# magic-research/vector_quantization

Measured on AMD Instinct MI355X. Metric: quantized tokens/sec, VQGAN quantizer forward K=16384 D=256, higher is better.
Workload: dtype f16+f32; 1 GPU; VQGAN K=16384 D=256, 256x256 images -> 16x16 tokens, bf16 latents, VQGANQuantizer.forward of the drop-in nn.Module, eval mode (prepare+argmin+gather+STE+loss); images_per_gpu=2048, parallelism=dp1 (independent shards, no data-path collective)

## Files before the change

vector_quantization_amd/csrc/vqhip.hip:

```cpp
#include "vqhip.h"

#include <hip/hip_runtime.h>
#include <stdio.h>
#include <string.h>

#include "vqhip_host.h"
#include "vqhip_kernels.h"
#include "vqhip_prepare_kernels.h"
#include "vqhip_proposal_kernels.h"
#include "vqhip_refine_kernels.h"
#include "vqhip_proposal32_kernels.h"
#include "vqhip_exact_kernels.h"
#include "vqhip_stream_kernels.h"
#include "vqhip_update_kernels.h"
#include "vqhip_sort_kernels.h"
#include "vqhip_aux_kernels.h"
#include "vqhip_exchange_kernels.h"
#include "vqhip_step_kernels.h"
#include "vqhip_pool_kernels.h"
#include "vqhip_fsq_kernels.h"

#include <atomic>
#include <mutex>
#include <type_traits>
#include <vector>
static std::atomic<bool> g_prof_on{false};
static std::mutex g_prof_mu;
static std::vector<std::pair<hipEvent_t, hipEvent_t>> g_prof_events;
static size_t g_prof_used = 0;

static long prof_begin(hipStream_t s) {
    if (!g_prof_on.load(std::memory_order_relaxed)) return -1;
    std::lock_guard<std::mutex> lock(g_prof_mu);
    if (g_prof_used == g_prof_events.size()) {
        hipEvent_t a, b;
        if (hipEventCreate(&a) != hipSuccess || hipEventCreate(&b) != hipSuccess) { g_prof_on = false; return -1; }
        g_prof_events.emplace_back(a, b);
    }
    const long slot = (long)g_prof_used++;
    (void)hipEventRecord(g_prof_events[slot].first, s);
    return slot;
}
static void prof_end(long slot, hipStream_t s) {
    if (slot < 0) return;
    std::lock_guard<std::mutex> lock(g_prof_mu);
    if ((size_t)slot < g_prof_events.size()) (void)hipEventRecord(g_prof_events[slot].second, s);
}

static std::atomic<int> g_tune_slices{0};
static std::atomic<int> g_tune_force_exact{0};
static std::atomic<int> g_tune_stream{1};
#define VQ_FUSED_DECIDE_MAX_N 16384

template <int NSTEP, int TT, int WAVES, int TPS, int NBUF = 2, bool FILTER = false, bool NOAUX = false, bool GROUPS = false, int XD = 0>
static int launch_coarse_cfg(const char *ximg, int64_t N, const char *frag, int64_t nstages, int nslices, float *rec,
                             int64_t Np, const VqCbStats *cbst, const float *xh2, const float *rho2, int Dp, int metric,
                             const VqDecideOut &dec, int pad_stage, int tpb, hipStream_t s) {
    constexpr int LDS = NBUF * (TPS * NSTEP + VQ_AUX_CHUNKS(TPS)) * VQ_CHUNK_BYTES;
    auto kern = coarse_kernel<NSTEP, TT, WAVES, TPS, NBUF, FILTER, NOAUX, GROUPS, XD>;
    static LdsCache lds_set;
    if (int rc = ensure_dyn_lds((const void *)kern, LDS, lds_set)) return rc;
    const int64_t ntiles = (N + 15) / 16;
    const int64_t ntb = (ntiles + tpb - 1) / tpb;
    const int grid = (int)(ntb * nslices);
    const long slot = prof_begin(s);
    kern<<<grid, WAVES * 64, LDS, s>>>(ximg, N, frag, nstages, nslices, rec, Np, cbst, xh2, rho2, Dp, metric, dec, pad_stage, tpb);
    prof_end(slot, s);
    VQ_CHECK_LAUNCH("coarse_kernel");
    return VQHIP_OK;
}

template <int TT, int WAVES, int TPS, int NBUF, bool NOAUX, int KS>
static int launch_coarse32_cfg(const char *ximg, int64_t N, const char *frag, int64_t nstages, int nslices, float *rec,
                               int64_t Np, const VqCbStats *cbst, const float *xh2, const float *rho2, int Dp, int metric,
                               const int *n_dev, const VqGroupLists &grp, int pad_stage, int tpb, hipStream_t s) {
    constexpr int LDS = NBUF * (TPS * 2 + VQ_AUX_CHUNKS(TPS)) * VQ_CHUNK_BYTES;
    auto kern = coarse32_kernel<TT, WAVES, TPS, NBUF, NOAUX, KS, VQ_GROUP_TILES>;
    static LdsCache lds_set;
    if (int rc = ensure_dyn_lds((const void *)kern, LDS, lds_set)) return rc;
    const int64_t ntiles = (N + 15) / 16;
    const int64_t ntb = (ntiles + tpb - 1) / tpb;
    const long slot = prof_begin(s);
    kern<<<(int)(ntb * nslices), WAVES * 64, LDS, s>>>(ximg, N, frag, nstages, nslices, rec, Np, cbst, xh2, rho2, Dp, metric, n_dev, grp, pad_stage, tpb);
    prof_end(slot, s);
    VQ_CHECK_LAUNCH("coarse32_kernel");
    return VQHIP_OK;
}

template <int NSTEP, int TT, int WAVES, int TPS, int NBUF = 2, int XD = 0>
static int launch_rescan_cfg(const char *ximg, const char *frag, int64_t nstages, const int *rescan_list, const int *counters,
                             const float *thr, int *rescan_cnt, int *cand_list, hipStream_t s, const void *xrows = nullptr) {
    constexpr int LDS = NBUF * (TPS * NSTEP + VQ_AUX_CHUNKS(TPS)) * VQ_CHUNK_BYTES + WAVES * TT * 16 * 4 * (1 + VQ_RESCAN_LOCAL);
    auto kern = rescan_kernel<NSTEP, TT, WAVES, TPS, NBUF, XD>;
    static LdsCache lds_set;
    if (int rc = ensure_dyn_lds((const void *)kern, LDS, lds_set)) return rc;
    kern<<<256, WAVES * 64, LDS, s>>>(ximg, frag, nstages, rescan_list, counters, thr, rescan_cnt, cand_list, xrows);
    VQ_CHECK_LAUNCH("rescan_kernel");
    return VQHIP_OK;
}

#ifndef VQ_W32_MAX_D
#define VQ_W32_MAX_D 32
#endif
#ifndef VQ_NBUF_D32
#define VQ_NBUF_D32 4
#endif
#ifndef VQ_D32_SMALL_TT
#define VQ_D32_SMALL_TT 2
#define VQ_D32_SMALL_W 8
#endif
#ifndef VQ_MIN_SLICES_FILTER
#define VQ_MIN_SLICES_FILTER 1
#endif
static int balanced_tiles_per_block(int64_t N, int full) {
    if (full < 16) return full;
    const int64_t ntiles = (N + 15) / 16;
    int best = full;
    int64_t best_cost = ((ntiles + full - 1) / full + 255) / 256 * full;
    for (int tpb = full - 1; tpb >= full / 2 && tpb >= 8; --tpb) {
        const int64_t cost = ((ntiles + tpb - 1) / tpb + 255) / 256 * tpb;
        if (cost < best_cost) { best_cost = cost; best = tpb; }
    }
    return best;
}

static bool vq_xdirect(int64_t N, int64_t K, int D, int x_dtype, int metric, const int *n_dev) {
    if (D != 256 || n_dev != nullptr || vq_cb_layout(K, D).nstages < 2 || g_tune_slices.load() == 1) return false;
    if (x_dtype != VQHIP_DTYPE_BF16) return false;
    if (!vq_public_metric(metric)) return false;
    if (N <= VQ_FUSED_DECIDE_MAX_N) return false;
    return !(N <= 4096 || (N <= 256 * 64 && K <= 4096));
}
enum VqTokenSide { VQ_TOKENS_UNPREPARED, VQ_TOKENS_IMAGE, VQ_TOKENS_ROWS };

static int pick_slices(int64_t ntb, int64_t nstages, int min_slices = 2) {
    if (const int forced = g_tune_slices.load(); forced > 0) { int ns = forced; while (ns > 1 && ns > nstages) ns >>= 1; return ns; }
    int64_t want = (256 + ntb - 1) / ntb;
    want = want < min_slices ? min_slices : want;
    int ns = 1;
    while (ns < want && ns < VQ_MAX_SLICES) ns <<= 1;
    while (ns > 1 && ns > nstages) ns >>= 1;
    return ns;
}

struct VqGroupRun { int used, ks, noaux, pad_stage; };
static int launch_coarse(const char *ximg, int64_t N, const VqCbLayout &L, const char *frag, float *rec, int64_t Np,
                         const VqCbStats *cbst, const float *xh2, const float *rho2, int metric, const VqDecideOut &dec,
                         int *nslices_out, int *fused_decide_out, hipStream_t s, VqGroupLists grp = VqGroupLists{nullptr, nullptr, nullptr, nullptr, 0, 1, 0},
                         VqGroupRun *grun = nullptr, bool xd = false) {
    const int nstep = L.nstep;
    const bool small = N <= 256 * 64;
    const bool small16 = N <= 4096 || (N <= 256 * 64 && L.K <= 4096);
    const bool small32 = N < 512 * 512;
    const bool noaux = !VQ_IS_L2(metric);
    const int pad_stage = (L.K % ((int64_t)L.tps * VQ_TILE_CODES)) ? (int)(L.nstages - 1) : -1;
#define VQ_CFG(NS, TT, W, ...)                                                                      \
    {                                                                                               \
        int64_t ntb = (N + (W) * (TT) * 16 - 1) / ((W) * (TT) * 16);                                \
        int ns = pick_slices(ntb, L.nstages, (NS) <= 8 ? VQ_MIN_SLICES_FILTER : 2);                 \
        *nslices_out = ns;                                                                          \
        const int tpb = (ns == 1) ? balanced_tiles_per_block(N, (W) * (TT)) : (W) * (TT);           \
        VqDecideOut dsel = dec;                                                                     \
        if (!(ns == 1 || N <= VQ_FUSED_DECIDE_MAX_N)) dsel.idx = nullptr;                           \
        *fused_decide_out = dsel.idx != nullptr ? 1 : 0;                                            \
        return launch_coarse_cfg<NS, TT, W, __VA_ARGS__>(ximg, N, frag, L.nstages, ns, rec, Np, cbst, xh2, rho2, L.Dp, metric, dsel, pad_stage, tpb, s); \
    }
    switch (nstep) {
        case 2: if ((L.D <= 16 || (L.D <= VQ_W32_MAX_D && noaux)) && N >= VQ_W32_MIN_N && grp.bcnt != nullptr && grun != nullptr) {
                    const int tt = small32 ? 1 : 2;
                    const int full = 8 * tt * 2;
                    const int64_t ntb0 = (N + full * 16 - 1) / (full * 16);
                    int ns = pick_slices(ntb0, L.nstages, VQ_MIN_SLICES_FILTER);
                    ns = ns > VQ_GROUP_MAX_SLICES ? VQ_GROUP_MAX_SLICES : ns;
                    *nslices_out = ns;
                    int tpb = (ns == 1) ? balanced_tiles_per_block(N, full) : full;
                    tpb = (tpb + 1) & ~1;
                    *fused_decide_out = 0;
                    grun->used = 1; grun->ks = L.D <= 16 ? 1 : 2; grun->noaux = noaux ? 1 : 0; grun->pad_stage = pad_stage;
#define VQ_CFG32(TTW, NOAUXV, KSV) return launch_coarse32_cfg<TTW, 8, VQ_TPS_D32, VQ_NBUF_D32, NOAUXV, KSV>(ximg, N, frag, L.nstages, ns, rec, Np, cbst, xh2, rho2, L.Dp, metric, dec.n_dev, grp, pad_stage, tpb, s)
                    if (L.D <= 16) {
                        if (tt == 1) { if (noaux) VQ_CFG32(1, true, 1); else VQ_CFG32(1, false, 1); }
                        else { if (noaux) VQ_CFG32(2, true, 1); else VQ_CFG32(2, false, 1); }
                    } else {
                        if (tt == 1) { if (noaux) VQ_CFG32(1, true, 2); else VQ_CFG32(1, false, 2); }
                        else { if (noaux) VQ_CFG32(2, true, 2); else VQ_CFG32(2, false, 2); }
                    }
#undef VQ_CFG32
                }
                if (N >= VQ_GROUPS_MIN_N) {
                    if (noaux) { if (small32) VQ_CFG(2, VQ_D32_SMALL_TT, VQ_D32_SMALL_W, VQ_TPS_D32, VQ_NBUF_D32, true, true, true) else VQ_CFG(2, 4, 8, VQ_TPS_D32, VQ_NBUF_D32, true, true, true) }
                    if (small32) VQ_CFG(2, VQ_D32_SMALL_TT, VQ_D32_SMALL_W, VQ_TPS_D32, VQ_NBUF_D32, true, false, true) else VQ_CFG(2, 4, 8, VQ_TPS_D32, VQ_NBUF_D32, true, false, true)
                }
                if (noaux) { if (small32) VQ_CFG(2, VQ_D32_SMALL_TT, VQ_D32_SMALL_W, VQ_TPS_D32, VQ_NBUF_D32, true, true) else VQ_CFG(2, 4, 8, VQ_TPS_D32, VQ_NBUF_D32, true, true) }
                if (small32) VQ_CFG(2, VQ_D32_SMALL_TT, VQ_D32_SMALL_W, VQ_TPS_D32, VQ_NBUF_D32, true) else VQ_CFG(2, 4, 8, VQ_TPS_D32, VQ_NBUF_D32, true)
        case 4: if (small) VQ_CFG(4, 2, 8, 4, 4, true) else VQ_CFG(4, 4, 8, 4, 4, true)
        case 8: if (small) VQ_CFG(8, 2, 8, 4, 4, true) else VQ_CFG(8, 4, 8, 4, 4, true)
        case 16: if (xd && !small16) VQ_CFG(16, 4, 8, VQ_TPS16, 4, false, false, false, 1)
                 if (small16) VQ_CFG(16, 2, 8, VQ_TPS16, 4) else VQ_CFG(16, 4, 8, VQ_TPS16, 4)
        case 32: VQ_CFG(32, 2, 8, 2)
        case 48: VQ_CFG(48, 2, 8, 1)
        case 64: {
            auto cost = [&](int tokens, double eff) {
                const int64_t ntb = (N + tokens - 1) / tokens;
                const int ns = pick_slices(ntb, L.nstages, 2);
                return (double)((ntb * ns + 255) / 256) * tokens * ((double)L.nstages / ns) / eff;
            };
            if (cost(192, 1.18) < cost(128, 1.0)) VQ_CFG(64, 3, 4, 1) else VQ_CFG(64, 1, 8, 1)
        }
        default: break;
    }
#undef VQ_CFG
    return fail(VQHIP_EINVAL, "vqhip_argmin: unsupported padded D");
}

static int resident_grid(int per_cu) {
    static std::atomic<int> cus[VQ_MAX_DEVICES];
    int dev = 0, n = 0;
    if (hipGetDevice(&dev) != hipSuccess) return 256 * per_cu;
    if (dev >= 0 && dev < VQ_MAX_DEVICES && (n = cus[dev].load(std::memory_order_relaxed)) > 0) return n * per_cu;
    if (hipDeviceGetAttribute(&n, hipDeviceAttributeMultiprocessorCount, dev) != hipSuccess || n <= 0) n = 256;
    if (dev >= 0 && dev < VQ_MAX_DEVICES) cus[dev].store(n, std::memory_order_relaxed);
    return n * per_cu;
}

template <int MODE>
static int run_exact_tiled(const void *x, int x_dtype, const float *e, const float *en, const float *xn, int64_t N, int64_t K,
                           int D, int metric, u64 *keys, float *dout, hipStream_t s) {
    const int bf = x_dtype == VQHIP_DTYPE_F32 ? 0 : 1;
    const int64_t items = ((N + 127) / 128) * ((K + 255) / 256);
    if (g_tune_stream.load() && D % (bf ? 8 : 4) == 0 && items < (int64_t)1 << 31) {
        static LdsCache ssets[2];
        const int lds = vq_xs_lds_bytes(bf);
        const void *kern = bf ? (const void *)exact_stream_kernel<1, MODE> : (const void *)exact_stream_kernel<0, MODE>;
        if (int rc = ensure_dyn_lds(kern, lds, ssets[bf])) return rc;
        const int cap = resident_grid(2);
        const int grid = (int)(items < cap ? items : cap);
        if (bf) exact_stream_kernel<1, MODE><<<grid, 256, lds, s>>>(x, e, en, xn, N, K, D, metric, keys, dout);
        else exact_stream_kernel<0, MODE><<<grid, 256, lds, s>>>(x, e, en, xn, N, K, D, metric, keys, dout);
        VQ_CHECK_LAUNCH("exact_stream_kernel");
        return VQHIP_OK;
    }
    constexpr int LDS = 2 * 32 * 128 * 4 + 8 * 32 * 4;
    static LdsCache sets[4];
    const void *kerns[4] = {(const void *)exact_tiled_kernel<0, MODE, false>, (const void *)exact_tiled_kernel<1, MODE, false>,
                            (const void *)exact_tiled_kernel<0, MODE, true>, (const void *)exact_tiled_kernel<1, MODE, true>};
    const int v4 = (D % 4 == 0) ? 2 : 0;
    if (int rc = ensure_dyn_lds(kerns[v4 + bf], LDS, sets[v4 + bf])) return rc;
    int grid = (int)(items < 1024 ? items : 1024);
#define VQ_TILED(DT, V4) exact_tiled_kernel<DT, MODE, V4><<<grid, 256, LDS, s>>>(x, e, en, xn, N, K, D, metric, keys, dout)
    if (v4) { if (bf) VQ_TILED(1, true); else VQ_TILED(0, true); }
    else { if (bf) VQ_TILED(1, false); else VQ_TILED(0, false); }
#undef VQ_TILED
    VQ_CHECK_LAUNCH("exact_tiled_kernel");
    return VQHIP_OK;
}

template <int MODE>
static int exact_whole(const void *x, int x_dtype, const float *e, int64_t N, int64_t K, int D, int metric, const VqWsView &V,
                       int64_t *idx, float *dmin, int32_t *hist, float *dout, hipStream_t s) {
    constexpr bool keyed = MODE != 2;
    const bool l2 = metric == VQHIP_METRIC_L2;
    if (l2) if (int rc = vqhip_row_sqnorm(e, VQHIP_DTYPE_F32, K, D, V.en, s)) return rc;
    if constexpr (keyed) { fill_u64_kernel<<<256, 256, 0, s>>>(V.keys, N, ~0ull); VQ_CHECK_LAUNCH("fill_u64_kernel"); }
    if (l2) if (int rc = vqhip_row_sqnorm(x, x_dtype, N, D, V.xn_whole, s)) return rc;
    if (int rc = run_exact_tiled<MODE>(x, x_dtype, e, V.en, V.xn_whole, N, K, D, metric, keyed ? V.keys : nullptr, dout, s)) return rc;
    if constexpr (keyed) { finalize_kernel<<<256, 256, 0, s>>>(V.keys, nullptr, nullptr, N, idx, dmin, hist); VQ_CHECK_LAUNCH("finalize_kernel"); }
    return VQHIP_OK;
}

static int exact_few_max(int D) {
    if (D > 512 || D > VQ_FEW_MAX_D) return 0;
    static std::atomic<int> lds_limit{-1};
    int lim = lds_limit.load(std::memory_order_relaxed);
    if (lim < 0) {
        int dev = 0, v = 0;
        if (hipGetDevice(&dev) != hipSuccess || hipDeviceGetAttribute(&v, hipDeviceAttributeMaxSharedMemoryPerBlock, dev) != hipSuccess) v = 65536;
        lim = v;
        lds_limit.store(lim);
    }
    return vq_few_lds_bytes(D) <= lim ? VQ_EXACT_FEW_MAX : 0;
}

static int run_exact_rows(const void *x, int x_dtype, const float *e, const float *en, const float *xn, int64_t N, int64_t K, int D,
                          int metric, const int *row_list, const int *nrows_dev, u64 *keys, int *ticket, int64_t *idx,
                          int32_t *hist, hipStream_t s) {
    const int64_t ncb = (K + 63) / 64;
    const int grid = (int)(ncb < 256 ? 256 : (ncb > 1024 ? 1024 : ncb));
    if (D % 4) return fail(VQHIP_EINVAL, "exact_kernel: D % 4 != 0 (the proposal route has D % 8 == 0)");
    const int few_max = exact_few_max(D);
    const int lds = few_max ? vq_few_lds_bytes(D) : 0;
    static LdsCache sets[2];
    const int bf = x_dtype == VQHIP_DTYPE_F32 ? 0 : 1;
    if (int rc = ensure_dyn_lds(bf ? (const void *)exact_kernel<1> : (const void *)exact_kernel<0>, lds, sets[bf])) return rc;
    if (!bf)
        exact_kernel<0><<<grid, 256, lds, s>>>(x, e, en, xn, N, K, D, metric, row_list, nrows_dev, keys, ticket, idx, hist, few_max);
    else
        exact_kernel<1><<<grid, 256, lds, s>>>(x, e, en, xn, N, K, D, metric, row_list, nrows_dev, keys, ticket, idx, hist, few_max);
    VQ_CHECK_LAUNCH("exact_kernel");
    return VQHIP_OK;
}

template <int MODE>
static int run_segsum(const void *src, int x_dtype, const float *e, const int64_t *idx, const int32_t *order,
                      const int32_t *offsets, int64_t N, int64_t K, int D, const float *g_cb, float *dst, void *ws,
                      hipStream_t s) {
    float *partial = (float *)ws;
    const int64_t nranges = (N + VQ_SEG_RANGE - 1) / VQ_SEG_RANGE;
    int grid = (int)((nranges + 3) / 4); grid = grid < 1 ? 1 : (grid > 4096 ? 4096 : grid);
    if (x_dtype == VQHIP_DTYPE_F32) segsum_rows_kernel<MODE, 0><<<grid, 256, 0, s>>>(src, e, idx, order, offsets, N, (int)K, D, g_cb, dst, partial);
    else segsum_rows_kernel<MODE, 1><<<grid, 256, 0, s>>>(src, e, idx, order, offsets, N, (int)K, D, g_cb, dst, partial);
    VQ_CHECK_LAUNCH("segsum_rows_kernel");
    int fgrid = (int)((K + 3) / 4); fgrid = fgrid > 2048 ? 2048 : fgrid;
    segsum_fixup_kernel<<<fgrid, 256, 0, s>>>(offsets, (int)K, D, partial, dst);
    VQ_CHECK_LAUNCH("segsum_fixup_kernel");
    return VQHIP_OK;
}

static inline int vq_small_lanes(int D) { return D <= 8 ? 8 : (D <= 16 ? 16 : 32); }

template <bool NORMALIZE>
static int launch_row_small(const void *v, int dtype, int64_t R, int D, float eps, float *out, hipStream_t s) {
    const int L = vq_small_lanes(D);
    const int grid = waves_grid((R + 64 / L - 1) / (64 / L), 4);
#define VQ_ROW_SMALL(DT, LL) row_small_kernel<DT, LL, NORMALIZE><<<grid, 256, 0, s>>>(v, R, D, eps, out)
    if (dtype == VQHIP_DTYPE_F32) { if (L == 8) VQ_ROW_SMALL(0, 8); else if (L == 16) VQ_ROW_SMALL(0, 16); else VQ_ROW_SMALL(0, 32); }
    else { if (L == 8) VQ_ROW_SMALL(1, 8); else if (L == 16) VQ_ROW_SMALL(1, 16); else VQ_ROW_SMALL(1, 32); }
#undef VQ_ROW_SMALL
    VQ_CHECK_LAUNCH("row_small_kernel");
    return VQHIP_OK;
}

template <typename IdxT>
static int launch_hist(const IdxT *idx, int64_t N, int64_t K, int32_t *hist, void *stream) {
    constexpr bool i64 = sizeof(IdxT) == 8;
    VQ_REQUIRE(idx && hist && N >= 0 && K > 0, i64 ? "vqhip_hist: bad argument" : "vqhip_hist_i32: bad argument");
    if (N == 0) return VQHIP_OK;
    hipStream_t s = (hipStream_t)stream;
    if (K <= 32768 && N >= 16384) {
        static LdsCache lds_set;
        if (int rc = ensure_dyn_lds(i64 ? (const void *)hist_lds_kernel : (const void *)hist_i32_lds_kernel, (size_t)K * 4, lds_set)) return rc;
        int grid = (int)((N + 2047) / 2048); grid = grid > 256 ? 256 : grid;
        if constexpr (i64) hist_lds_kernel<<<grid, 1024, (size_t)K * 4, s>>>(idx, N, (int)K, hist);
        else hist_i32_lds_kernel<<<grid, 1024, (size_t)K * 4, s>>>(idx, N, (int)K, hist);
    } else {
        int grid = (int)((N + 255) / 256); grid = grid > 2048 ? 2048 : grid;
        if constexpr (i64) hist_kernel<<<grid, 256, 0, s>>>(idx, N, K, hist);
        else hist_i32_kernel<<<grid, 256, 0, s>>>(idx, N, K, hist);
    }
    VQ_CHECK_LAUNCH(i64 ? "hist_kernel" : "hist_i32_kernel");
    return VQHIP_OK;
// ... 1285 lines not shown
```

vector_quantization_amd/csrc/vqhip_proposal_kernels.h:

```cpp
#pragma once
#include "vqhip_kernels.h"
struct Top2 { float v1, v2, v3; uint32_t c1, c2; };
__device__ __forceinline__ float row_margin(const VqCbStats *st, int Dp, int metric, float X2, float R2, float *bf16_part = nullptr);

struct VqDecideOut {
    int64_t *idx; int32_t *hist;
    int *rescan_list, *multi_list, *exact_list, *counters;
    u64 *keys; float *thr_out; int *rescan_cnt;
    int *arrive;
    const int *n_dev;
    const void *xrows; float *xh2_w, *rho2_w, *xn_w;
};
template <bool AGENT>
__device__ __forceinline__ void decide_rows(int64_t n, bool oob, const VqCbStats *st, int Dp, int metric, int nslices,
                                            const float *rec, const float *xh2, const float *rho2, int64_t Np,
                                            const VqDecideOut &o, int *wcount, int *wbase, const float *rece2 = nullptr);

__device__ __forceinline__ void top_insert(Top2 &t, float v, uint32_t c) {
    if (v > t.v1) { t.v3 = fmaxf(t.v3, t.v2); t.v2 = t.v1; t.c2 = t.c1; t.v1 = v; t.c1 = c; }
    else if (v > t.v2) { t.v3 = fmaxf(t.v3, t.v2); t.v2 = v; t.c2 = c; }
    else t.v3 = fmaxf(t.v3, v);
}

__device__ __forceinline__ void top_merge_lane(Top2 &t, int xor_mask) {
    Top2 o;
    o.v1 = __shfl_xor(t.v1, xor_mask, 64); o.v2 = __shfl_xor(t.v2, xor_mask, 64); o.v3 = __shfl_xor(t.v3, xor_mask, 64);
    o.c1 = __shfl_xor(t.c1, xor_mask, 64); o.c2 = __shfl_xor(t.c2, xor_mask, 64);
    if (o.c1 != 0xFFFFFFFFu) top_insert(t, o.v1, o.c1);
    if (o.c2 != 0xFFFFFFFFu) top_insert(t, o.v2, o.c2);
    t.v3 = fmaxf(t.v3, o.v3);
}

__device__ __forceinline__ int tile_row16(int e, int lane) { return 16 * (e >> 2) + 4 * (lane >> 4) + (e & 3); }

#ifndef VQ_D32_PLAIN_OCC
#define VQ_D32_PLAIN_OCC 2
#endif
template <int NSTEP, int TT, int WAVES, int TPS, int NBUF = 2, bool FILTER = false, bool NOAUX = false,
          bool GROUPS = false, int XD = 0>
__global__ __launch_bounds__(WAVES * 64, (FILTER && NSTEP <= 2) ? (GROUPS ? 4 : VQ_D32_PLAIN_OCC) : WAVES / 4) void coarse_kernel(
    const char *__restrict__ ximg, int64_t N, const char *__restrict__ frag, int64_t nstages, int nslices,
    float *__restrict__ rec, int64_t Np, const VqCbStats *__restrict__ cbst, const float *__restrict__ xh2,
    const float *__restrict__ rho2, int Dp, int metric, VqDecideOut dec, int pad_stage, int tpb) {
    extern __shared__ __attribute__((aligned(16))) char lds[];
    static_assert(NSTEP % 2 == 0, "16x16x32 layout: 32-dim k-steps");
    static_assert(!GROUPS || FILTER, "group records are a form of the filtered epilogue");
    constexpr bool GBRANCH = TT >= VQ_GROUP_BRANCH_MIN_TT;
    constexpr bool PIPE = (TPS % 2) == 0;
    constexpr bool PIPE_H = (TPS == 1) && (WAVES <= 4);
    static_assert(!(PIPE_H && (NOAUX || FILTER)), "half-tile ping-pong: plain large-D form only");
    constexpr int NS32 = NSTEP / 2;
    constexpr int NCH = TPS * NSTEP + VQ_AUX_CHUNKS(TPS);
    constexpr int STAGE_BYTES = NCH * VQ_CHUNK_BYTES;
    constexpr int NE = 8;
#ifndef VQ_SCALAR_WAVE
#define VQ_SCALAR_WAVE 1
#endif
    const int lane = threadIdx.x & 63;
    const int wave = (VQ_SCALAR_WAVE && NSTEP > 2) ? __builtin_amdgcn_readfirstlane((int)(threadIdx.x >> 6)) : (int)(threadIdx.x >> 6);
    const int64_t ntt = (N + 31) / 32 * 2;
    if (dec.n_dev != nullptr) {
        const int64_t nd = *dec.n_dev;
        N = nd < N ? nd : N;
        if ((int64_t)(blockIdx.x / nslices) * tpb * 16 >= N) return;
    }
    const bool wave_active = wave * TT < tpb;
    cb_stats_publish(cbst);
    const int sl = blockIdx.x % nslices;
    const int64_t tb = blockIdx.x / nslices;
    const int64_t st0 = (nstages * sl) / nslices, st1 = (nstages * (sl + 1)) / nslices;
  for (bool once = true; once; once = false) {

    half8 xf[TT][NS32];
    if constexpr (XD == 0) {
#pragma unroll
        for (int t = 0; t < TT; ++t) {
            int64_t tt = tb * tpb + wave * TT + t;
            tt = tt < ntt ? tt : ntt - 1;
            const char *src = ximg + tt * (int64_t)(NS32 * VQ_CHUNK_BYTES) + lane * 16;
#pragma unroll
            for (int s = 0; s < NS32; ++s) xf[t][s] = *(const half8 *)(src + s * VQ_CHUNK_BYTES);
        }
    } else {
        static_assert(XD == 1 && !FILTER && !GROUPS && !NOAUX && (NSTEP % 4) == 0, "token side in the prologue: bf16 rows, plain D % 64 == 0 forms");
        const int q4 = lane >> 4, r16 = lane & 15;
        constexpr int Dr = NS32 * 32;
        static_assert(NS32 == 8 && NBUF >= 4 && 2 * STAGE_BYTES >= WAVES * 16 * 528, "row tile: D = 256, staged behind stage 1");
        char *stg = lds + 2 * STAGE_BYTES + wave * (16 * 528);
        const int hr = lane >> 5, c32 = lane & 31;
#pragma unroll
        for (int t = 0; t < TT; ++t) {
            const int64_t tok0 = (tb * tpb + wave * TT + t) * 16;
#pragma unroll
            for (int i = 0; i < 8; ++i) {
                const int64_t tok = tok0 + 2 * i + hr;
                const int64_t trow = tok < N ? tok : N - 1;
                xf[t][i] = *(const half8 *)((const uint16_t *)dec.xrows + trow * Dr + 8 * c32);
            }
        }
        __builtin_amdgcn_sched_barrier(0);
#pragma unroll
        for (int t = 0; t < TT; ++t) {
#pragma unroll
            for (int i = 0; i < 8; ++i) *(half8 *)(stg + (2 * i + hr) * 528 + 16 * c32) = xf[t][i];
#pragma unroll
            for (int s = 0; s < NS32; ++s) xf[t][s] = *(const half8 *)(stg + r16 * 528 + 64 * s + 16 * q4);
        }
#pragma unroll
        for (int t = 0; t < TT; ++t) {
            const int64_t tok = (tb * tpb + wave * TT + t) * 16 + r16;
            [[maybe_unused]] const int64_t trow = tok < N ? tok : N - 1;
            const bool stats = sl == 0;
            float sh[2] = {0.0f, 0.0f}, sr[2] = {0.0f, 0.0f}, pn[2][8];
#pragma unroll
            for (int j = 0; j < 8; ++j) { pn[0][j] = 0.0f; pn[1][j] = 0.0f; }
#pragma unroll
            for (int s = 0; s < NS32; ++s) {
                float v[8];
                half8 f;
                typedef uint32_t u32x4 __attribute__((ext_vector_type(4)));
                typedef _Float16 half2v __attribute__((ext_vector_type(2)));
                typedef float float2v __attribute__((ext_vector_type(2)));
                const u32x4 bits = __builtin_bit_cast(u32x4, xf[t][s]);
#pragma unroll
                for (int j = 0; j < 4; ++j) {
                    const uint32_t lo = bits[j] << 16, hi = bits[j] & 0xFFFF0000u;
                    v[2 * j] = __uint_as_float(lo); v[2 * j + 1] = __uint_as_float(hi);
                    float2v c;
                    c[0] = (lo & 0x7FFFFFFFu) < 0x38800000u ? 0.0f : v[2 * j];
                    c[1] = (hi & 0x7FFFFFFFu) < 0x38800000u ? 0.0f : v[2 * j + 1];
                    const half2v h = __builtin_convertvector(c, half2v);
                    f[2 * j] = h[0]; f[2 * j + 1] = h[1];
                }
                if (stats) {
#pragma unroll
                    for (int j = 0; j < 8; ++j) {
                        const float b = (float)f[j], res = v[j] - b;
                        sh[s & 1] = fmaf(b, b, sh[s & 1]); sr[s & 1] = fmaf(res, res, sr[s & 1]);
                        pn[s & 1][j] = fmaf(v[j], v[j], pn[s & 1][j]);
                    }
                }
                xf[t][s] = f;
            }
            if (!stats) continue;
            float a = 0.0f, b = 0.0f;
#pragma unroll
            for (int g = 0; g < 8; ++g) {
                a += __shfl(sh[g >> 2], (g & 3) * 16 + r16, 64);
                b += __shfl(sr[g >> 2], (g & 3) * 16 + r16, 64);
            }
            float q[8];
#pragma unroll
            for (int j = 0; j < 8; ++j) q[j] = pn[0][j] + pn[1][j];
#pragma unroll
            for (int j = 0; j < 8; ++j) q[j] = q[j] + __shfl_xor(q[j], 32, 64);
#pragma unroll
            for (int j = 0; j < 8; ++j) q[j] = q[j] + __shfl_xor(q[j], 16, 64);
            float a0 = q[0] + q[4], a1 = q[1] + q[5], a2 = q[2] + q[6], a3 = q[3] + q[7];
            a0 = a0 + a2; a1 = a1 + a3;
            a0 = a0 + a1;
            if (sl == 0 && q4 == 0 && tok < N && wave * TT + t < tpb) { dec.xh2_w[tok] = a; dec.rho2_w[tok] = b; dec.xn_w[tok] = a0; }
        }
    }
    if constexpr (PIPE_H) {
#pragma unroll
        for (int t = 0; t < TT; ++t)
#pragma unroll
            for (int s = 0; s < NS32; ++s) {
                if (t >= TT / 2) asm volatile("" : "+a"(xf[t][s]));
                else asm volatile("" : "+v"(xf[t][s]));
            }
    }

    float b1[TT], b2[TT], th[TT], mg[TT];
    uint32_t t1[TT];
#pragma unroll
    for (int t = 0; t < TT; ++t) { b1[t] = -INFINITY; b2[t] = -INFINITY; th[t] = -INFINITY; mg[t] = INFINITY; t1[t] = 0; }
    static_assert(!FILTER || PIPE, "the filtered epilogue is written for the ping-pong form");
    float sc0 = 0.0f, sc1 = 0.0f, sc2 = 0.0f;
    if constexpr (FILTER) {
        const VqCbStats stv = cb_stats_view(cbst);
#pragma unroll
        for (int t = 0; t < TT; ++t) {
            int64_t tokn = (tb * tpb + wave * TT + t) * 16 + (lane & 15);
            tokn = tokn < N ? tokn : N - 1;
            const float m = row_margin(&stv, Dp, metric, xh2[tokn], rho2[tokn]);
            mg[t] = (m > 0.0f) ? m : INFINITY;
        }
    }

    auto issue_stage = [&](int64_t st, int buf) {
        const char *src = frag + st * (int64_t)STAGE_BYTES;
        char *dstb = lds + buf * STAGE_BYTES;
        for (int c = wave; c < NCH; c += WAVES)
            __builtin_amdgcn_global_load_lds(
                (const __attribute__((address_space(1))) void *)(src + c * VQ_CHUNK_BYTES + lane * 16),
                (__attribute__((address_space(3))) void *)(dstb + c * VQ_CHUNK_BYTES), 16, 0, 0);
    };

    constexpr int AHEAD = NBUF >= 3 ? 2 : 1;
#ifndef VQ_LAG_MIN_STAGES
#define VQ_LAG_MIN_STAGES 48
#endif
    const int lag = (NBUF >= 4 && wave >= WAVES / 2 && st1 - st0 >= VQ_LAG_MIN_STAGES) ? 1 : 0;
    if (st0 < st1) issue_stage(st0, 0);
    if (AHEAD >= 2 && st0 + 1 < st1) issue_stage(st0 + 1, 1);
    vq_dma_barrier();

    f32x4 accA[2][TT], accB[2][TT];
#pragma unroll
    for (int c = 0; c < 2; ++c)
#pragma unroll
        for (int t = 0; t < TT; ++t)
#pragma unroll
            for (int q = 0; q < 4; ++q)
                accB[c][t][q] = GROUPS ? -INFINITY : -3.0e38f;
    if constexpr (PIPE_H) {
#pragma unroll
        for (int t = 0; t < TT; ++t) accA[1][t] = f32x4{-3.0e38f, -3.0e38f, -3.0e38f, -3.0e38f};
    }

    for (int64_t it = st0; it < st1 + ((NBUF >= 4 && st1 - st0 >= VQ_LAG_MIN_STAGES) ? 1 : 0); ++it) {
        if (it + AHEAD < st1) issue_stage(it + AHEAD, (int)((it + AHEAD - st0) % NBUF));
        const int64_t st = it - lag;
        if (st < st0 || st >= st1 || !wave_active) { vq_dma_barrier(); continue; }
        const int buf = (int)((st - st0) % NBUF);
        const char *base = lds + buf * STAGE_BYTES;
        const char *aux = base + TPS * NSTEP * VQ_CHUNK_BYTES;
      auto run_stage = [&](auto with_aux_tag) __attribute__((always_inline)) {
        constexpr bool WITH_AUX = decltype(with_aux_tag)::value;
        if constexpr (PIPE_H) {
            constexpr int PFH = VQ_PIPEH_PF;
            constexpr int TOTALH = 4 * TT;
            const uint32_t tile = (uint32_t)st;
#pragma unroll
            for (int c = 0; c < 2; ++c) {
                const f32x4 a4 = *(const f32x4 *)(aux + (16 * c + 4 * (lane >> 4)) * 4);
                uint32_t old[TT];
#pragma unroll
                for (int t = 0; t < TT; ++t) { accA[c][t] = a4; old[t] = __float_as_uint(b1[t]); }
                half8 af[PFH + 1];
#pragma unroll
                for (int i = 0; i < PFH; ++i) af[i] = *(const half8 *)(base + (2 * i + c) * VQ_CHUNK_BYTES + lane * 16);
#pragma unroll
                for (int s = 0; s < NS32; ++s) {
                    if (s + PFH < NS32)
                        af[(s + PFH) % (PFH + 1)] = *(const half8 *)(base + (2 * (s + PFH) + c) * VQ_CHUNK_BYTES + lane * 16);
#pragma unroll
                    for (int t = 0; t < TT; ++t)
                        accA[c][t] = __builtin_amdgcn_mfma_f32_16x16x32_f16(af[s % (PFH + 1)], xf[t][s], accA[c][t], 0, 0, 0);
#pragma unroll
                    for (int id = s * TOTALH / NS32; id < (s + 1) * TOTALH / NS32; ++id) {
                        const int t = id / 4, q = id % 4, e = 4 * (1 - c) + q;
                        float v = __uint_as_float((__float_as_uint(accA[1 - c][t][q]) & 0xFFFFFFF0u) | (uint32_t)e);
                        b2[t] = __builtin_amdgcn_fmed3f(b1[t], b2[t], v);
                        b1[t] = vmax(b1[t], v);
                    }
                    __builtin_amdgcn_sched_barrier(0);
                }
                const uint32_t tgp = tile - (c == 0 ? 1u : 0u);
#pragma unroll
                for (int t = 0; t < TT; ++t) t1[t] = (__float_as_uint(b1[t]) != old[t]) ? tgp : t1[t];
            }
        } else {
#ifndef VQ_PF_TT2
#define VQ_PF_TT2 3
#endif
#ifndef VQ_PF_TT4
#define VQ_PF_TT4 2
#endif
#ifndef VQ_CHUNK_SB
#define VQ_CHUNK_SB 2
#endif
#ifndef VQ_STAGE_PF
#define VQ_STAGE_PF 1
#endif
        constexpr bool CHUNK_SB = NSTEP >= 4 && NSTEP <= 16 && !FILTER && (VQ_CHUNK_SB == 2 || (VQ_CHUNK_SB == 1 && TT <= 2));
        constexpr int PF = NSTEP <= 32 ? (CHUNK_SB ? (TT <= 2 ? VQ_PF_TT2 : VQ_PF_TT4) : 1) : (NSTEP <= 48 ? 2 : 4);
        constexpr bool STAGE_PF = (VQ_STAGE_PF != 0) && CHUNK_SB && TPS >= 2;
        half8 af[PF + 1];
#pragma unroll
        for (int ti = 0; ti < TPS; ++ti) {
            f32x4 (&cur)[2][TT] = (PIPE && (ti & 1)) ? accB : accA;
            f32x4 (&prv)[2][TT] = (PIPE && (ti & 1)) ? accA : accB;
            if constexpr (WITH_AUX) {
#pragma unroll
                for (int c = 0; c < 2; ++c) {
                    f32x4 a4 = *(const f32x4 *)(aux + (ti * 32 + 16 * c + 4 * (lane >> 4)) * 4);
#pragma unroll
                    for (int t = 0; t < TT; ++t) cur[c][t] = a4;
                }
            }
            uint32_t old[TT];
#pragma unroll
            for (int t = 0; t < TT; ++t) old[t] = __float_as_uint(b1[t]);
            constexpr int RING = PF + 1;
            const int g0 = STAGE_PF ? ti * NSTEP : 0;
            if (!STAGE_PF || ti == 0) {
#pragma unroll
                for (int i = 0; i < PF; ++i)
                    if (i < NSTEP) af[i] = *(const half8 *)(base + (ti * NSTEP + i) * VQ_CHUNK_BYTES + lane * 16);
            }
#pragma unroll
            for (int ch = 0; ch < NSTEP; ++ch) {
                if (ch + PF < NSTEP || (STAGE_PF && ti + 1 < TPS))
                    af[(g0 + ch + PF) % RING] = *(const half8 *)(base + (ti * NSTEP + ch + PF) * VQ_CHUNK_BYTES + lane * 16);
#pragma unroll
                for (int t = 0; t < TT; ++t) {
                    if constexpr (!WITH_AUX) {
                        if (ch < 2) {
                            cur[ch & 1][t] = __builtin_amdgcn_mfma_f32_16x16x32_f16(af[(g0 + ch) % RING], xf[t][ch >> 1], f32x4{0.0f, 0.0f, 0.0f, 0.0f}, 0, 0, 0);
                            continue;
                        }
                    }
                    cur[ch & 1][t] = __builtin_amdgcn_mfma_f32_16x16x32_f16(af[(g0 + ch) % RING], xf[t][ch >> 1], cur[ch & 1][t], 0, 0, 0);
                }
                if constexpr (FILTER) {
                    const uint32_t tgp = (uint32_t)(st * TPS + ti) - 1u;
#pragma unroll
                    for (int i = 0; i < (TT + NSTEP - 1) / NSTEP; ++i) {
                        constexpr int EVERY = (NSTEP / TT) > 0 ? NSTEP / TT : 1;
                        const int t = (TT >= NSTEP) ? ch * (TT / NSTEP) + i : ((ch % EVERY == 0) ? ch / EVERY : -1);
                        if (t >= 0 && t < TT) {
                            float after[TT];
#pragma unroll
                            for (int u = 0; u < TT; ++u) after[u] = cur[ch & 1][u][0];
                            tile_max8<TT>(sc0, sc1, sc2, prv[0][t], prv[1][t], after);
                            if constexpr (GROUPS) {
                                if (!GBRANCH || __any(!(sc0 < th[t]))) {
                                    const float nb = vmax(b1[t], sc0);
                                    b2[t] = __builtin_amdgcn_fmed3f(b1[t], b2[t], sc0);
                                    t1[t] = (__float_as_uint(nb) != __float_as_uint(b1[t])) ? tgp : t1[t];
                                    b1[t] = nb;
                                }
                            } else if (__any(!(sc0 < th[t]))) {
                                const uint32_t was = __float_as_uint(b1[t]);
#pragma unroll
                                for (int e = 0; e < NE; ++e) {
                                    float v = __uint_as_float((__float_as_uint(prv[e >> 2][t][e & 3]) & 0xFFFFFFF0u) | (uint32_t)e);
                                    b2[t] = __builtin_amdgcn_fmed3f(b1[t], b2[t], v);
                                    b1[t] = vmax(b1[t], v);
                                }
                                t1[t] = (__float_as_uint(b1[t]) != was) ? tgp : t1[t];
                            }
                        }
                    }
                }
                constexpr int TOTAL = NE * TT;
                constexpr bool RETIRE = PIPE && !FILTER;
#pragma unroll
                for (int i = 0; RETIRE && i < (TOTAL + NSTEP - 1) / NSTEP; ++i) {
                    constexpr int EVERY = (NSTEP / TOTAL) > 0 ? NSTEP / TOTAL : 1;
                    const int id = (TOTAL >= NSTEP) ? ch * (TOTAL / NSTEP) + i : ((ch % EVERY == 0) ? ch / EVERY : -1);
                    if (id >= 0 && id < TOTAL) {
                        const int t = id / NE, e = id % NE;
                        float v = __uint_as_float((__float_as_uint(prv[e >> 2][t][e & 3]) & 0xFFFFFFF0u) | (uint32_t)e);
                        b2[t] = __builtin_amdgcn_fmed3f(b1[t], b2[t], v);
                        b1[t] = vmax(b1[t], v);
                    }
                }
                if constexpr (CHUNK_SB) __builtin_amdgcn_sched_barrier(0);
            }
            if constexpr (!PIPE && !PIPE_H) {
#pragma unroll
                for (int t = 0; t < TT; ++t)
#pragma unroll
                    for (int e = 0; e < NE; ++e) {
                        float v = __uint_as_float((__float_as_uint(cur[e >> 2][t][e & 3]) & 0xFFFFFFF0u) | (uint32_t)e);
                        b2[t] = __builtin_amdgcn_fmed3f(b1[t], b2[t], v);
                        b1[t] = vmax(b1[t], v);
                    }
            }
            if constexpr (!FILTER) {
                const uint32_t tgp = (uint32_t)(st * TPS + ti) - (PIPE ? 1u : 0u);
#pragma unroll
                for (int t = 0; t < TT; ++t)
                    t1[t] = (__float_as_uint(b1[t]) != old[t]) ? tgp : t1[t];
            }
        }
        }
      };
        if constexpr (NOAUX) {
            if (st == (int64_t)pad_stage) run_stage(std::true_type{}); else run_stage(std::false_type{});
        } else {
            run_stage(std::true_type{});
        }
        if constexpr (FILTER && (!GROUPS || GBRANCH)) {
#pragma unroll
            for (int t = 0; t < TT; ++t) th[t] = quad_rows_max(b1[t]) - mg[t];
        }
        vq_dma_barrier();
    }
    if (PIPE_H && st1 > st0) {
#pragma unroll
        for (int t = 0; t < TT; ++t) {
            const uint32_t old = __float_as_uint(b1[t]);
#pragma unroll
            for (int q = 0; q < 4; ++q) {
                float v = __uint_as_float((__float_as_uint(accA[1][t][q]) & 0xFFFFFFF0u) | (uint32_t)(4 + q));
                b2[t] = __builtin_amdgcn_fmed3f(b1[t], b2[t], v);
                b1[t] = vmax(b1[t], v);
            }
            t1[t] = (__float_as_uint(b1[t]) != old) ? (uint32_t)(st1 * TPS - 1) : t1[t];
        }
    }
    if (PIPE && st1 > st0) {
#pragma unroll
        for (int t = 0; t < TT; ++t) {
            const uint32_t old = __float_as_uint(b1[t]);
            if constexpr (GROUPS) {
                float g = accB[0][t][0];
#pragma unroll
                for (int e = 1; e < NE; ++e) g = __builtin_amdgcn_fmed3f(g, accB[e >> 2][t][e & 3], INFINITY);
                b2[t] = __builtin_amdgcn_fmed3f(b1[t], b2[t], g);
                b1[t] = vmax(b1[t], g);
            } else {
#pragma unroll
                for (int e = 0; e < NE; ++e) {
                    float v = __uint_as_float((__float_as_uint(accB[e >> 2][t][e & 3]) & 0xFFFFFFF0u) | (uint32_t)e);
                    b2[t] = __builtin_amdgcn_fmed3f(b1[t], b2[t], v);
                    b1[t] = vmax(b1[t], v);
                }
            }
            t1[t] = (__float_as_uint(b1[t]) != old) ? (uint32_t)(st1 * TPS - 1) : t1[t];
        }
    }

    bool ident[TT];
#pragma unroll
    for (int t = 0; t < TT; ++t) ident[t] = true;
    if constexpr (GROUPS) {
        auto bound_up = [](float v) {
            const uint32_t b = __float_as_uint(v);
            return __uint_as_float((b & 0x80000000u) ? (b & 0xFFFFFFF0u) : (b | 0xFu));
        };
        constexpr int RB = NSTEP <= 2 ? VQ_REPLAY_BATCH : (NSTEP <= 4 ? 2 : 1);
#pragma unroll
        for (int t = 0; t < TT; ++t) {
            const float top = quad_rows_max(b1[t]);
            const int64_t tokn = (tb * tpb + wave * TT + t) * 16 + (lane & 15);
            const bool need = (mg[t] < INFINITY) && (b1[t] > -INFINITY) && !(b1[t] < top - mg[t]) && tokn < N && wave * TT + t < tpb &&
                              t1[t] >= (uint32_t)(st0 * TPS) && t1[t] < (uint32_t)(st1 * TPS);
            float e1 = -INFINITY, e2 = -INFINITY;
            u64 todo = __ballot(need);
            while (todo) {
                uint32_t T[RB];
                u64 rest = todo;
#pragma unroll
                for (int i = 0; i < RB; ++i) {
                    const int l = rest ? (__ffsll((unsigned long long)rest) - 1) : (__ffsll((unsigned long long)todo) - 1);
                    T[i] = (uint32_t)__builtin_amdgcn_readlane((int)t1[t], l);
                    rest &= rest - 1;
                }
                half8 a[RB][NSTEP];
                f32x4 acc[RB][2];
#pragma unroll
                for (int i = 0; i < RB; ++i) {
                    const int64_t rst = T[i] / TPS;
                    const int rti = (int)(T[i] % TPS);
                    const char *sb = frag + rst * (int64_t)STAGE_BYTES;
#pragma unroll
                    for (int ch = 0; ch < NSTEP; ++ch)
                        a[i][ch] = *(const half8 *)(sb + (rti * NSTEP + ch) * VQ_CHUNK_BYTES + lane * 16);
#pragma unroll
                    for (int c = 0; c < 2; ++c) {
                        if (NOAUX && rst != (int64_t)pad_stage) acc[i][c] = f32x4{0.0f, 0.0f, 0.0f, 0.0f};
                        else acc[i][c] = *(const f32x4 *)(sb + TPS * NSTEP * VQ_CHUNK_BYTES + (rti * 32 + 16 * c + 4 * (lane >> 4)) * 4);
                    }
                }
                u64 done = 0;
#pragma unroll
                for (int i = 0; i < RB; ++i) {
#pragma unroll
                    for (int ch = 0; ch < NSTEP; ++ch)
                        acc[i][ch & 1] = __builtin_amdgcn_mfma_f32_16x16x32_f16(a[i][ch], xf[t][ch >> 1], acc[i][ch & 1], 0, 0, 0);
                    float w1 = -INFINITY, w2 = -INFINITY;
#pragma unroll
                    for (int e = 0; e < NE; ++e) {
                        float v = __uint_as_float((__float_as_uint(acc[i][e >> 2][e & 3]) & 0xFFFFFFF0u) | (uint32_t)e);
                        w2 = __builtin_amdgcn_fmed3f(w1, w2, v);
                        w1 = vmax(w1, v);
                    }
                    const bool mine = need && t1[t] == T[i];
                    e1 = mine ? w1 : e1; e2 = mine ? w2 : e2;
                    done |= __ballot(mine);
                }
                todo &= ~done;
            }
            const float other = bound_up(b2[t]);
            if (need) { b1[t] = e1; b2[t] = fmaxf(other, e2); }
            else { b2[t] = fmaxf(other, bound_up(b1[t])); }
            ident[t] = need;
        }
    }

#pragma unroll
    for (int t = 0; t < TT; ++t) {
        Top2 r; r.v1 = r.v2 = r.v3 = -INFINITY; r.c1 = r.c2 = 0xFFFFFFFFu;
        {
            uint32_t bits = __float_as_uint(b1[t]);
            uint32_t code = t1[t] * 32u + (uint32_t)tile_row16((int)(bits & 7u), lane);
            if (ident[t] && b1[t] > -INFINITY) top_insert(r, b1[t], code);
            r.v3 = fmaxf(r.v3, b2[t]);
        }
        top_merge_lane(r, 16);
        top_merge_lane(r, 32);
        const int64_t tokn = (tb * tpb + wave * TT + t) * 16 + (lane & 15);
        if (lane < 16 && tokn < N && wave * TT + t < tpb) {
            float *rp = rec + (int64_t)sl * VQ_REC_FIELDS * Np + tokn;
            if (dec.idx != nullptr && nslices > 1) {
                __hip_atomic_store(rp, r.v1, __ATOMIC_RELAXED, __HIP_MEMORY_SCOPE_AGENT);
                __hip_atomic_store(rp + Np, __uint_as_float(r.c1), __ATOMIC_RELAXED, __HIP_MEMORY_SCOPE_AGENT);
                __hip_atomic_store(rp + 2 * Np, r.v2, __ATOMIC_RELAXED, __HIP_MEMORY_SCOPE_AGENT);
                __hip_atomic_store(rp + 3 * Np, __uint_as_float(r.c2), __ATOMIC_RELAXED, __HIP_MEMORY_SCOPE_AGENT);
                __hip_atomic_store(rp + 4 * Np, r.v3, __ATOMIC_RELAXED, __HIP_MEMORY_SCOPE_AGENT);
            } else {
                rp[0] = r.v1; rp[Np] = __uint_as_float(r.c1); rp[2 * Np] = r.v2;
                rp[3 * Np] = __uint_as_float(r.c2); rp[4 * Np] = r.v3;
            }
        }
    }

    if (dec.idx != nullptr) {
        int *flags = (int *)lds;
        asm volatile("s_waitcnt vmcnt(0)" ::: "memory");
        __syncthreads();
        if (threadIdx.x == 0) {
            int last = 1;
            if (nslices > 1) {
                last = (atomicAdd(&dec.arrive[tb], 1) == nslices - 1) ? 1 : 0;
            }
            flags[0] = last;
        }
        __syncthreads();
        const bool last = flags[0] != 0;
        __syncthreads();
        if (last) {
            int *wcount = (int *)lds, *wbase = wcount + 3 * 16;
            int64_t n = tb * (int64_t)(tpb * 16) + threadIdx.x;
            const bool oob = (int)threadIdx.x >= tpb * 16 || n >= N;
            if (n >= N) n = N - 1;
            decide_rows<true>(n, oob, cbst, Dp, metric, nslices, rec, xh2, rho2, Np, dec, wcount, wbase);
        }
    }
  }
}
```

Measured before the change: 160.4 million tokens/s.

## Run both codebook slices in one workgroup with in-kernel decide for row-direct path

Adds an XD==2 coarse-kernel form in which a single workgroup walks all codebook stages, flushes its half-codebook top-2 record at the midpoint, then runs the decide step directly without cross-workgroup atomics or arrival counters. It is chosen when the two-slice grid would not fill more waves than the one-workgroup grid. The aim is to remove reloading the token tile per slice, the atomic arrival handshake, and the separate decide pass. In exchange each workgroup runs twice as long and the grid has half as many workgroups, which may hurt load balance. The previous XD==1 path also stops fusing decide.

```diff
diff --git a/vector_quantization_amd/csrc/vqhip.hip b/vector_quantization_amd/csrc/vqhip.hip
--- a/vector_quantization_amd/csrc/vqhip.hip
+++ b/vector_quantization_amd/csrc/vqhip.hip
@@ -62,7 +62,7 @@
     if (int rc = ensure_dyn_lds((const void *)kern, LDS, lds_set)) return rc;
     const int64_t ntiles = (N + 15) / 16;
     const int64_t ntb = (ntiles + tpb - 1) / tpb;
-    const int grid = (int)(ntb * nslices);
+    const int grid = (int)(ntb * (XD == 2 ? 1 : nslices));
     const long slot = prof_begin(s);
     kern<<<grid, WAVES * 64, LDS, s>>>(ximg, N, frag, nstages, nslices, rec, Np, cbst, xh2, rho2, Dp, metric, dec, pad_stage, tpb);
     prof_end(slot, s);
@@ -133,7 +133,15 @@
 }
 enum VqTokenSide { VQ_TOKENS_UNPREPARED, VQ_TOKENS_IMAGE, VQ_TOKENS_ROWS };
 
-static int pick_slices(int64_t ntb, int64_t nstages, int min_slices = 2) {
+static int pick_slices(int64_t ntb, int64_t nstages, int min_slices = 2);
+static bool vq_one_workgroup(int64_t N, int64_t nstages) {
+    if (g_tune_slices.load() > 0) return false;
+    const int64_t ntb = (N + 511) / 512;
+    if (nstages < 2 || pick_slices(ntb, nstages) != 2) return false;
+    return 2 * ((ntb + 255) / 256) <= (2 * ntb + 255) / 256;
+}
+
+static int pick_slices(int64_t ntb, int64_t nstages, int min_slices) {
     if (const int forced = g_tune_slices.load(); forced > 0) { int ns = forced; while (ns > 1 && ns > nstages) ns >>= 1; return ns; }
     int64_t want = (256 + ntb - 1) / ntb;
     want = want < min_slices ? min_slices : want;
@@ -195,7 +203,22 @@
                 if (small32) VQ_CFG(2, VQ_D32_SMALL_TT, VQ_D32_SMALL_W, VQ_TPS_D32, VQ_NBUF_D32, true) else VQ_CFG(2, 4, 8, VQ_TPS_D32, VQ_NBUF_D32, true)
         case 4: if (small) VQ_CFG(4, 2, 8, 4, 4, true) else VQ_CFG(4, 4, 8, 4, 4, true)
         case 8: if (small) VQ_CFG(8, 2, 8, 4, 4, true) else VQ_CFG(8, 4, 8, 4, 4, true)
-        case 16: if (xd && !small16) VQ_CFG(16, 4, 8, VQ_TPS16, 4, false, false, false, 1)
+        case 16: if (xd && !small16) {
+                     const int tpb = 8 * 4;
+                     VqDecideOut dsel = dec;
+                     if (L.nstages >= 2 && vq_one_workgroup(N, L.nstages)) {
+                         *nslices_out = 2;
+                         *fused_decide_out = 1;
+                         return launch_coarse_cfg<16, 4, 8, VQ_TPS16, 4, false, false, false, 2>(ximg, N, frag, L.nstages, 2, rec, Np, cbst, xh2, rho2, L.Dp, metric, dsel, pad_stage, tpb, s);
+                     }
+                     if (L.nstages < 2) return fail(VQHIP_EINVAL, "vqhip_argmin: the row-direct proposal form needs two stages");
+                     int ns = pick_slices((N + tpb * 16 - 1) / (tpb * 16), L.nstages, 2);
+                     ns = ns < 2 ? 2 : ns;
+                     *nslices_out = ns;
+                     dsel.idx = nullptr;
+                     *fused_decide_out = 0;
+                     return launch_coarse_cfg<16, 4, 8, VQ_TPS16, 4, false, false, false, 1>(ximg, N, frag, L.nstages, ns, rec, Np, cbst, xh2, rho2, L.Dp, metric, dsel, pad_stage, tpb, s);
+                 }
                  if (small16) VQ_CFG(16, 2, 8, VQ_TPS16, 4) else VQ_CFG(16, 4, 8, VQ_TPS16, 4)
         case 32: VQ_CFG(32, 2, 8, 2)
         case 48: VQ_CFG(48, 2, 8, 1)
diff --git a/vector_quantization_amd/csrc/vqhip_proposal_kernels.h b/vector_quantization_amd/csrc/vqhip_proposal_kernels.h
--- a/vector_quantization_amd/csrc/vqhip_proposal_kernels.h
+++ b/vector_quantization_amd/csrc/vqhip_proposal_kernels.h
@@ -66,9 +66,11 @@
     }
     const bool wave_active = wave * TT < tpb;
     cb_stats_publish(cbst);
-    const int sl = blockIdx.x % nslices;
-    const int64_t tb = blockIdx.x / nslices;
-    const int64_t st0 = (nstages * sl) / nslices, st1 = (nstages * (sl + 1)) / nslices;
+    constexpr bool ONEWG = XD == 2;
+    const int sl = ONEWG ? 0 : blockIdx.x % nslices;
+    const int64_t tb = ONEWG ? blockIdx.x : blockIdx.x / nslices;
+    const int64_t st0 = ONEWG ? 0 : (nstages * sl) / nslices, st1 = ONEWG ? nstages : (nstages * (sl + 1)) / nslices;
+    [[maybe_unused]] const int64_t mid = nstages / 2;
   for (bool once = true; once; once = false) {
 
     half8 xf[TT][NS32];
@@ -82,7 +84,7 @@
             for (int s = 0; s < NS32; ++s) xf[t][s] = *(const half8 *)(src + s * VQ_CHUNK_BYTES);
         }
     } else {
-        static_assert(XD == 1 && !FILTER && !GROUPS && !NOAUX && (NSTEP % 4) == 0, "token side in the prologue: bf16 rows, plain D % 64 == 0 forms");
+        static_assert((XD == 1 || XD == 2) && !FILTER && !GROUPS && !NOAUX && (NSTEP % 4) == 0, "token side in the prologue: bf16 rows, plain D % 64 == 0 forms");
         const int q4 = lane >> 4, r16 = lane & 15;
         constexpr int Dr = NS32 * 32;
         static_assert(NS32 == 8 && NBUF >= 4 && 2 * STAGE_BYTES >= WAVES * 16 * 528, "row tile: D = 256, staged behind stage 1");
@@ -202,7 +204,7 @@
 #ifndef VQ_LAG_MIN_STAGES
 #define VQ_LAG_MIN_STAGES 48
 #endif
-    const int lag = (NBUF >= 4 && wave >= WAVES / 2 && st1 - st0 >= VQ_LAG_MIN_STAGES) ? 1 : 0;
+    const int lag = (NBUF >= 4 && wave >= WAVES / 2 && (ONEWG ? mid : st1 - st0) >= VQ_LAG_MIN_STAGES) ? 1 : 0;
     if (st0 < st1) issue_stage(st0, 0);
     if (AHEAD >= 2 && st0 + 1 < st1) issue_stage(st0 + 1, 1);
     vq_dma_barrier();
@@ -220,10 +222,41 @@
         for (int t = 0; t < TT; ++t) accA[1][t] = f32x4{-3.0e38f, -3.0e38f, -3.0e38f, -3.0e38f};
     }
 
-    for (int64_t it = st0; it < st1 + ((NBUF >= 4 && st1 - st0 >= VQ_LAG_MIN_STAGES) ? 1 : 0); ++it) {
+    for (int64_t it = st0; it < st1 + ((NBUF >= 4 && (ONEWG ? mid : st1 - st0) >= VQ_LAG_MIN_STAGES) ? 1 : 0); ++it) {
         if (it + AHEAD < st1) issue_stage(it + AHEAD, (int)((it + AHEAD - st0) % NBUF));
         const int64_t st = it - lag;
         if (st < st0 || st >= st1 || !wave_active) { vq_dma_barrier(); continue; }
+        if constexpr (ONEWG) {
+            if (st == mid) {
+                int hl = lane;
+                asm volatile("" : "+v"(hl));
+#pragma unroll
+                for (int t = 0; t < TT; ++t) {
+                    const uint32_t old = __float_as_uint(b1[t]);
+#pragma unroll
+                    for (int e = 0; e < NE; ++e) {
+                        float v = __uint_as_float((__float_as_uint(accB[e >> 2][t][e & 3]) & 0xFFFFFFF0u) | (uint32_t)e);
+                        b2[t] = __builtin_amdgcn_fmed3f(b1[t], b2[t], v);
+                        b1[t] = vmax(b1[t], v);
+                    }
+                    t1[t] = (__float_as_uint(b1[t]) != old) ? (uint32_t)(mid * TPS - 1) : t1[t];
+                    Top2 r; r.v1 = r.v2 = r.v3 = -INFINITY; r.c1 = r.c2 = 0xFFFFFFFFu;
+                    if (b1[t] > -INFINITY) top_insert(r, b1[t], t1[t] * 32u + (uint32_t)tile_row16((int)(__float_as_uint(b1[t]) & 7u), hl));
+                    r.v3 = fmaxf(r.v3, b2[t]);
+                    top_merge_lane(r, 16);
+                    top_merge_lane(r, 32);
+                    const int64_t tokn = (tb * tpb + wave * TT + t) * 16 + (hl & 15);
+                    if (hl < 16 && tokn < N && wave * TT + t < tpb) {
+                        float *rp = rec + tokn;
+                        rp[0] = r.v1; rp[Np] = __uint_as_float(r.c1); rp[2 * Np] = r.v2;
+                        rp[3 * Np] = __uint_as_float(r.c2); rp[4 * Np] = r.v3;
+                    }
+                    b1[t] = -INFINITY; b2[t] = -INFINITY; t1[t] = 0;
+#pragma unroll
+                    for (int c = 0; c < 2; ++c) accB[c][t] = f32x4{-3.0e38f, -3.0e38f, -3.0e38f, -3.0e38f};
+                }
+            }
+        }
         const int buf = (int)((st - st0) % NBUF);
         const char *base = lds + buf * STAGE_BYTES;
         const char *aux = base + TPS * NSTEP * VQ_CHUNK_BYTES;
@@ -507,8 +540,8 @@
         top_merge_lane(r, 32);
         const int64_t tokn = (tb * tpb + wave * TT + t) * 16 + (lane & 15);
         if (lane < 16 && tokn < N && wave * TT + t < tpb) {
-            float *rp = rec + (int64_t)sl * VQ_REC_FIELDS * Np + tokn;
-            if (dec.idx != nullptr && nslices > 1) {
+            float *rp = rec + (int64_t)(ONEWG ? 1 : sl) * VQ_REC_FIELDS * Np + tokn;
+            if (!ONEWG && dec.idx != nullptr && nslices > 1) {
                 __hip_atomic_store(rp, r.v1, __ATOMIC_RELAXED, __HIP_MEMORY_SCOPE_AGENT);
                 __hip_atomic_store(rp + Np, __uint_as_float(r.c1), __ATOMIC_RELAXED, __HIP_MEMORY_SCOPE_AGENT);
                 __hip_atomic_store(rp + 2 * Np, r.v2, __ATOMIC_RELAXED, __HIP_MEMORY_SCOPE_AGENT);
@@ -521,7 +554,15 @@
         }
     }
 
-    if (dec.idx != nullptr) {
+    if constexpr (ONEWG) {
+        asm volatile("s_waitcnt vmcnt(0)" ::: "memory");
+        __syncthreads();
+        int *wcount = (int *)lds, *wbase = wcount + 3 * 16;
+        int64_t n = tb * (int64_t)(tpb * 16) + threadIdx.x;
+        const bool oob = (int)threadIdx.x >= tpb * 16 || n >= N;
+        if (n >= N) n = N - 1;
+        decide_rows<true>(n, oob, cbst, Dp, metric, 2, rec, dec.xh2_w, dec.rho2_w, Np, dec, wcount, wbase);
+    } else if (XD != 1 && dec.idx != nullptr) {
         int *flags = (int *)lds;
         asm volatile("s_waitcnt vmcnt(0)" ::: "memory");
         __syncthreads();
```

Result: faster. 162.3 million tokens/s (median of 6 runs) (+1.2%).
